# phazei/ComfyUI-HunyuanVideo-Foley

Measured on AMD Instinct MI355X. Metric: audio-sec/sec (5s clip, 50-step Euler, CFG 4.5), higher is better.
Workload: dtype bf16; 1 GPU; c2: T2A 5 s, 50 Euler steps, CFG 4.5, hunyuanvideo-foley-xxl, bs=1/GPU, bf16 GEMM operands / fp32 accumulate, weight storage none, DAC-VAE fp32 decode to 48 kHz, host-to-host (H2D noise + D2H waveform timed); clips_per_gpu=1, parallelism=dp1, hip_graph=True, progress_callback=False, collectives=0, bundle_bytes=10565004032, rccl_nranks=1

## Files before the change

comfyui-hunyuanvideo-foley_amd/csrc/common.h:

```cpp
#pragma once
#include <hip/hip_runtime.h>
#include <hip/hip_ext.h>
#include <stdint.h>

#include <atomic>

typedef __attribute__((ext_vector_type(16))) float f32x16;
typedef __attribute__((ext_vector_type(4))) float f32x4;
typedef __attribute__((ext_vector_type(8))) __bf16 bf16x8;
typedef __attribute__((ext_vector_type(4))) unsigned int u32x4;
typedef uint16_t bf16_t;
typedef _Float16 f16_t;
typedef __attribute__((ext_vector_type(8))) _Float16 f16x8;

enum { FOLEY_F32 = 0, FOLEY_BF16 = 1, FOLEY_I32 = 2, FOLEY_F8E4M3 = 3, FOLEY_F8E5M2 = 4, FOLEY_F16 = 5 };
__host__ __device__ constexpr bool foley_is_half(int dt) { return dt == FOLEY_BF16 || dt == FOLEY_F16; }

__device__ __forceinline__ float bf16_to_f32(bf16_t v) { return __uint_as_float(((uint32_t)v) << 16); }
__device__ __forceinline__ bf16_t f32_to_bf16(float f) {
  uint32_t u = __float_as_uint(f);
  if ((u & 0x7fffffffu) > 0x7f800000u) return (bf16_t)((u >> 16) | 0x40);
  u += 0x7fffu + ((u >> 16) & 1u);
  return (bf16_t)(u >> 16);
}
// ... 108 lines not shown
  float scale;
  int per;
  int dense_from;
  int dense_base;
};

__host__ __device__ __forceinline__ int rb_nearest_exact(int l, float scale, int Ls) {
  const int s = (int)floorf(((float)l + 0.5f) * scale);
  return s < Ls ? s : Ls - 1;
}

__device__ __forceinline__ const float* rb_row(const RowBcast& b, int r) {
  const float* p = b.p;
  if (b.step_ptr) p += (long)(*b.step_ptr) * b.step_stride;
  if (b.mode == 1) p += ((long)(r / b.rows_per_cfg) * b.L + (r % b.L)) * b.ld;
  else if (b.mode == 2) {
    const int s = rb_nearest_exact(r % b.L, b.scale, b.Ls), cfg = r / b.rows_per_cfg;
    const int idx = cfg < b.dense_from ? cfg * b.per + (s & (b.per - 1)) : b.dense_base + (cfg - b.dense_from) * b.Ls + s;
    p += (long)idx * b.ld;
  }
  return p;
}

struct FoleyProfHook {
  hipEvent_t e0, e1;
  const void* fn;
};
extern thread_local FoleyProfHook g_foley_prof;
#define FOLEY_LAUNCH(kernel, grid, block, lds, st, ...)                                                          \
  do {                                                                                                           \
    if (g_foley_prof.e0) {                                                                                       \
      hipExtLaunchKernelGGL(kernel, grid, block, lds, st, g_foley_prof.e0, g_foley_prof.e1, 0, __VA_ARGS__);     \
      g_foley_prof.e0 = nullptr;                                                                                 \
      g_foley_prof.fn = (const void*)(kernel);                                                                   \
    } else {                                                                                                     \
      hipLaunchKernelGGL(kernel, grid, block, lds, st, __VA_ARGS__);                                             \
    }                                                                                                            \
  } while (0)

#define FOLEY_CHECK_HIP(expr)                                         \
  do {                                                                \
    hipError_t _e = (expr);                                           \
    if (_e != hipSuccess) return foley_set_err(hipGetErrorString(_e), __FILE__, __LINE__); \
  } while (0)

int foley_set_err(const char* msg, const char* file, int line);
// ... 10 lines not shown
```

comfyui-hunyuanvideo-foley_amd/csrc/foley_rt.hip:

```cpp
#include "../../include/foley_hip.h"
#include "kernels.h"
#include "gemm_plan.h"

#include <algorithm>
#include <climits>
#include <cmath>
#include <cstdio>
#include <cstdlib>
#include <cstring>
#include <cxxabi.h>
#include <atomic>
#include <mutex>
#include <string>
#include <type_traits>
#include <unordered_map>
#include <vector>

thread_local FoleyProfHook g_foley_prof = {nullptr, nullptr};

static std::mutex g_setup_mutex;

static thread_local std::string g_err;
int foley_set_err(const char* msg, const char* file, int line) {
  const char* base = strrchr(file, '/');
// ... 1633 lines not shown
                     {Cout}, &an));
      GemmArgs g = gemm_plain(S_in, clips * Tout, down, X, Cout);
      g.lda = C; g.segV = Tout; g.segS = Tin; g.taps = 2 * s; g.tapC = C; g.dil = 1; g.tap0 = -pad; g.rstride = s;
      g.out1 = S_alt; g.alpha = (const float*)an; g.alphaC = Cout;
      TRY(launch_gemm(g, FOLEY_F32, EPI_DAC, 0, st));
      std::swap(S_in, S_alt);
    }
    Tin = Tout;
    C = Cout;
  }
  {
    Lin co, qc;
    TRY(get_lin(c, "enc.out", FOLEY_F32, L, 3 * C, true, &co));
    TRY(get_lin(c, "enc.qc", FOLEY_F32, 2 * L, L, true, &qc));
    TRY(launch_gemm(gemm_conv(S_in, clips * Tin, Tin, C, 3, 1, co, Z0, L), FOLEY_F32, EPI_STORE_F32, 0, st));
    TRY(launch_gemm(gemm_plain(Z0, clips * Tin, qc, Z1, 2 * L), FOLEY_F32, EPI_STORE_F32, 0, st));
    TRY(launch_rows_to_planes(Z1, clips, Tin, 2 * L, params, st));
  }
  HIPTRY(hipEventRecord(c->ev1, st));
  c->timed = true;
  return 0;
}

static RowBcast to_rb(const foley_rowbcast* r) {
  if (!r || !r->p) return rb_none();
  const int L = r->L > 0 ? r->L : 1, Ls = r->mode == 2 ? (r->Ls > 0 ? r->Ls : 1) : 0;
  const int per = (r->mode == 2 && r->period > 0 && !(r->period & (r->period - 1))) ? r->period : 0;
  RowBcast b{r->p, (long)r->ld, r->mode, r->rows_per_cfg > 0 ? r->rows_per_cfg : 1, L, nullptr, 0, Ls, Ls ? (float)Ls / (float)L : 0.f, per, 0, 0};
  if (per > 0) {
    b.dense_from = r->periodic_cfgs > 0 ? r->periodic_cfgs : INT_MAX;
    b.dense_base = r->periodic_cfgs > 0 ? r->periodic_cfgs * per : 0;
  }
  return b;
}

static int gemm_args_of(const foley_gemm_desc* d, GemmArgs& g) {
  if (!d) return FAIL(FOLEY_ERR_INVALID, "null descriptor");
  g = GemmArgs{};
  g.A = d->A; g.W = d->W; g.bias = d->bias; g.M = d->M; g.N = d->N; g.K = d->K; g.lda = d->lda;
  g.segV = d->segV; g.segS = d->segS; g.taps = d->taps; g.tapC = d->tapC; g.dil = d->dil; g.tap0 = d->tap0;
  g.out0 = d->out0; g.out1 = d->out1; g.osegV = d->osegV; g.out_seg = d->out_seg; g.out_row = d->out_row;
  g.out_shift = d->out_shift; g.out_check = d->out_check; g.rb = to_rb(&d->rb); g.res = d->res;
  g.alpha = d->alpha; g.alphaC = d->alphaC > 0 ? d->alphaC : 1;
  g.ksplit = d->ksplit;
  g.rstride = d->rstride;
  g.ldw = d->ldw;
  g.wfmt = d->wfmt;
  g.gelu_erf = d->gelu_erf;
  if (d->partials) {
    if (d->partial_slabs < 1) return FAIL(FOLEY_ERR_INVALID, "partials need partial_slabs >= 1");
    g.partials = d->partials; g.partial_stride = (long)d->M * d->N; g.partial_cap = d->partial_slabs;
    g.partial_half = d->partial_dtype != 0;
    if (d->partial_dtype != 0 && d->partial_dtype != d->dtype) return FAIL(FOLEY_ERR_INVALID, "partial_dtype must be 0 (fp32) or the operand dtype");
  }
  if (g.segV < 1 || g.segS < 1 || g.osegV < 1 || g.taps < 1) return FAIL(FOLEY_ERR_INVALID, "bad GEMM descriptor");
  if (d->epilogue == EPI_QKV_SPLIT) {
// ... 248 lines not shown
extern "C" int foley_op_windows_stitch(const float* x, int clips, int n_win, int C, int L, int Ltot, const int32_t* starts,
                                       const float* weights, float* out, void* stream) {
  return launch_windows_stitch(x, clips, n_win, C, L, Ltot, starts, weights, out, (hipStream_t)stream);
}

extern "C" int foley_op_flow_mix(const float* noise, const float* x0, int x0_clips, int clips, int C, int L, float sigma,
                                 float* out, void* stream) {
  return launch_flow_mix(noise, x0, x0_clips, clips, C, L, sigma, out, (hipStream_t)stream);
}

extern "C" int foley_op_latent_rows(const float* x, int clips, int C, int L, int ncfg, void* out, int out_dtype,
                                    void* stream) {
  return launch_latent_rows(x, clips, C, L, ncfg, out, out_dtype, (hipStream_t)stream);
}

extern "C" int foley_op_dac_out(const float* s, const float* w, const float* bias, int B, int T, int C, float* out,
                                void* stream) {
  return launch_dac_out(s, w, bias, B, T, C, out, (hipStream_t)stream);
}

extern "C" int foley_op_rows_add_act(const float* a, const float* v, int R, int D, int act_silu, void* out, int out_dtype,
                                     void* stream) {
  if (!out || R < 1 || D < 1) return FAIL(FOLEY_ERR_INVALID, "rows_add_act: null output or empty problem");
  return launch_rows_add_act(a, v ? rb_vec(v, 0, nullptr) : rb_none(), R, D, act_silu ? 1 : 0, out, out_dtype, (hipStream_t)stream);
}

extern "C" int foley_op_add_periodic(const float* x, const float* pos, int R, int D, int period, void* out, int out_dtype,
                                     void* stream) {
  if (!x || !pos || !out || R < 1 || D < 1 || period < 1) return FAIL(FOLEY_ERR_INVALID, "add_periodic: null argument or empty problem");
  return launch_add_periodic(x, pos, R, D, period, out, out_dtype, (hipStream_t)stream);
}

extern "C" int foley_op_gather_rows(const float* src, const int32_t* idx, int n_idx, int groups, int src_rows, int D, float* out,
                                    void* stream) {
  if (!src || !idx || !out || n_idx < 1 || groups < 1 || src_rows < 1 || D < 1)
    return FAIL(FOLEY_ERR_INVALID, "gather_rows: null argument or empty problem");
  return launch_gather_rows(src, idx, n_idx, groups, src_rows, D, out, (hipStream_t)stream);
}

extern "C" int foley_op_cast(const void* src, int src_dtype, void* dst, int dst_dtype, long n, void* stream) {
  if (!src || !dst || n < 1) return FAIL(FOLEY_ERR_INVALID, "cast: null argument or empty problem");
  return launch_cast(src, src_dtype, dst, dst_dtype, n, (hipStream_t)stream);
}

extern "C" int foley_op_rows_periodic_check(const float* x, int groups, int rows, int period, int D, int32_t* flags, void* stream) {
  if (!x || !flags || groups < 1 || rows < 1 || period < 1 || D < 1)
    return FAIL(FOLEY_ERR_INVALID, "rows_periodic_check: null argument or empty problem");
// ... 41 lines not shown
```

comfyui-hunyuanvideo-foley_amd/csrc/rowops.hip:

```cpp
#include <type_traits>

#include "kernels.h"

namespace {

#define FOLEY_LAUNCH_CHECK()                                                             \
  do {                                                                                   \
    hipError_t _e = hipGetLastError();                                                   \
    if (_e != hipSuccess) return foley_set_err(hipGetErrorString(_e), __FILE__, __LINE__); \
  } while (0)

template <typename OutT> struct Pack4;
template <> struct Pack4<float> {
  static __device__ __forceinline__ void store(float* p, const f32x4 v) { *(f32x4*)p = v; }
};
template <> struct Pack4<bf16_t> {
  static __device__ __forceinline__ void store(bf16_t* p, const f32x4 v) {
    uint2 w;
    w.x = pack_bf16x2(v[0], v[1]);
    w.y = pack_bf16x2(v[2], v[3]);
    *(uint2*)p = w;
  }
};

template <> struct Pack4<f16_t> {
  static __device__ __forceinline__ void store(f16_t* p, const f32x4 v) {
    uint2 w;
    w.x = pack_f16x2(v[0], v[1]);
    w.y = pack_f16x2(v[2], v[3]);
    *(uint2*)p = w;
  }
};

template <typename ST> __device__ __forceinline__ f32x4 slab_load4(const void* base, long elem) {
  if constexpr (sizeof(ST) == 4) {
    return *(const f32x4*)((const float*)base + elem);
  } else {
    const uint2 w = *(const uint2*)((const ST*)base + elem);
    const ST* h = (const ST*)&w;
    f32x4 v = {Cvt<ST>::from(h[0]), Cvt<ST>::from(h[1]), Cvt<ST>::from(h[2]), Cvt<ST>::from(h[3])};
    return v;
  }
}

struct LnPair {
  LnArgs a[2];
  int blocks0;
  long long* dbg;
};
static long long* g_ln_dbg = nullptr;
extern "C" void foley_debug_ln_timeline(void* p) { g_ln_dbg = (long long*)p; }

template <typename OutT, int MAXV, bool PEND, bool SLAB16 = false>
__global__ __launch_bounds__(128) void ln_mod_kernel(const LnPair pr, int D, float eps) {
  using ST = typename std::conditional<SLAB16, OutT, float>::type;
  const int sel = (int)blockIdx.x >= pr.blocks0 ? 1 : 0;
  const LnArgs& A = pr.a[sel];
  float* __restrict__ x = A.x;
  const int M = A.M;
  const RowBcast& shift = A.shift;
  const RowBcast& scale = A.scale;
  OutT* __restrict__ out = (OutT*)A.out;
  const int row = ((int)blockIdx.x - (sel ? pr.blocks0 : 0)) * 2 + (threadIdx.x >> 6);
  const int lane = threadIdx.x & 63;
  if (row >= M) return;
  const int nv = D >> 2;
  f32x4* xr = (f32x4*)(x + (long)row * D);
  const f32x4* sh = shift.p ? (const f32x4*)rb_row(shift, row) : nullptr;
  const f32x4* sc = scale.p ? (const f32x4*)rb_row(scale, row) : nullptr;
  const f32x4 z4 = {0.f, 0.f, 0.f, 0.f};
  f32x4 v[MAXV], hv[MAXV], cv[MAXV];
#pragma unroll
  for (int i = 0; i < MAXV; ++i) {
    const int c = min(lane + i * 64, nv - 1);
    v[i] = xr[c];
    hv[i] = sh ? sh[c] : z4;
    cv[i] = sc ? sc[c] : z4;
// ... 47 lines not shown
#pragma unroll
      for (int u = 0; u < 4; ++u) {
        const float d = v[i][u] - mean;
        q += d * d;
      }
    }
  const float rstd = 1.0f / sqrtf(wave_sum(q) / (float)D + eps);
  OutT* orow = out + (long)row * D;
#pragma unroll
  for (int i = 0; i < MAXV; ++i) {
    const int c = lane + i * 64;
    if (c < nv) {
      f32x4 y;
#pragma unroll
      for (int u = 0; u < 4; ++u) y[u] = (v[i][u] - mean) * rstd * (1.0f + cv[i][u]) + hv[i][u];
      Pack4<OutT>::store(orow + c * 4, y);
    }
  }
}

#ifndef FOLEY_LN_RPB
#define FOLEY_LN_RPB 1
#endif
template <typename OutT, int MAXV, bool PEND, int WPR, int SEL, bool SLAB16>
__device__ __forceinline__ void ln_mod_wide_body(const LnPair& pr, int D, float eps) {
  using ST = typename std::conditional<SLAB16, OutT, float>::type;
  constexpr int RPB = FOLEY_LN_RPB;
  __shared__ float red[RPB][2][WPR];
  constexpr int sel = SEL;
  const LnArgs& A = pr.a[SEL];
  const int M = A.M;
  const int wave = threadIdx.x >> 6, lane = threadIdx.x & 63;
  const int rb = wave / WPR, part = wave % WPR;
  const int row_u = ((int)blockIdx.x - (sel ? pr.blocks0 : 0)) * RPB + rb;
  const bool live = row_u < M;
  const int row = live ? row_u : M - 1;
  const int c0 = part * (MAXV * 64) + lane;
  const bool stamp = pr.dbg && threadIdx.x == 0;
  if (stamp) pr.dbg[(long)blockIdx.x * 4 + 0] = wall_clock64();
  f32x4* xr = (f32x4*)(A.x + (long)row * D);
  const f32x4* sh = A.shift.p ? (const f32x4*)rb_row(A.shift, row) : nullptr;
  const f32x4* sc = A.scale.p ? (const f32x4*)rb_row(A.scale, row) : nullptr;
  const f32x4 z4 = {0.f, 0.f, 0.f, 0.f};
  f32x4 v[MAXV], hv[MAXV], cv[MAXV];
#pragma unroll
  for (int i = 0; i < MAXV; ++i) {
    const int c = c0 + i * 64;
    v[i] = xr[c];
    hv[i] = sh ? sh[c] : z4;
    cv[i] = sc ? sc[c] : z4;
  }
  if (PEND && A.pend.partials) {
    constexpr int SB = 6;
    const LnPending& P = A.pend;
    const f32x4* gp = (const f32x4*)rb_row(P.gate, row);
    const f32x4* bp = (const f32x4*)P.bias;
    f32x4 acc[MAXV], gt[MAXV];
#pragma unroll
    for (int i = 0; i < MAXV; ++i) {
      const int c = c0 + i * 64;
      gt[i] = gp[c];
      acc[i] = bp ? bp[c] : z4;
// ... 3 lines not shown
#pragma unroll
      for (int u = 0; u < SB; ++u) {
        const int s = min(s0 + u, P.k - 1);
        const long pe = s * P.stride + (long)row * D;
#pragma unroll
        for (int i = 0; i < MAXV; ++i) t[u][i] = slab_load4<ST>(P.partials, pe + 4L * (c0 + i * 64));
      }
#pragma unroll
      for (int u = 0; u < SB; ++u) {
        const float w = (s0 + u < P.k) ? 1.0f : 0.0f;
#pragma unroll
        for (int i = 0; i < MAXV; ++i)
#pragma unroll
          for (int e = 0; e < 4; ++e) acc[i][e] += w * t[u][i][e];
      }
    }
#pragma unroll
    for (int i = 0; i < MAXV; ++i) {
#pragma unroll
      for (int e = 0; e < 4; ++e) v[i][e] += gt[i][e] * acc[i][e];
      if (live) xr[c0 + i * 64] = v[i];
    }
  }
  if (pr.dbg) {
    asm volatile("s_waitcnt vmcnt(0)" ::: "memory");
    if (stamp) pr.dbg[(long)blockIdx.x * 4 + 1] = wall_clock64();
  }
  float s = 0.f;
#pragma unroll
  for (int i = 0; i < MAXV; ++i) s += (v[i][0] + v[i][1]) + (v[i][2] + v[i][3]);
  s = wave_sum(s);
  const float nw = (float)(MAXV * 4 * 64);
  const float mean_w = s / nw;
  float q = 0.f;
#pragma unroll
  for (int i = 0; i < MAXV; ++i)
#pragma unroll
    for (int u = 0; u < 4; ++u) {
      const float d = v[i][u] - mean_w;
      q += d * d;
    }
  q = wave_sum(q);
  if (lane == 0) {
    red[rb][0][part] = s;
    red[rb][1][part] = q;
  }
  __syncthreads();
  float tot = 0.f;
#pragma unroll
  for (int w = 0; w < WPR; ++w) tot += red[rb][0][w];
  const float mean = tot / (float)D;
  float qt = 0.f;
#pragma unroll
  for (int w = 0; w < WPR; ++w) {
    const float dm = red[rb][0][w] / nw - mean;
    qt += red[rb][1][w] + nw * dm * dm;
  }
  const float rstd = 1.0f / sqrtf(qt / (float)D + eps);
  if (stamp) pr.dbg[(long)blockIdx.x * 4 + 2] = wall_clock64();
  if (!live) return;
  OutT* orow = (OutT*)A.out + (long)row * D;
#pragma unroll
  for (int i = 0; i < MAXV; ++i) {
    f32x4 y;
#pragma unroll
    for (int u = 0; u < 4; ++u) y[u] = (v[i][u] - mean) * rstd * (1.0f + cv[i][u]) + hv[i][u];
    Pack4<OutT>::store(orow + (c0 + i * 64) * 4, y);
  }
  if (stamp) pr.dbg[(long)blockIdx.x * 4 + 3] = wall_clock64();
}

template <typename OutT, int MAXV, bool PEND, int WPR, bool SLAB16 = false>
__global__ __launch_bounds__(64 * FOLEY_LN_RPB * WPR) void ln_mod_wide_kernel(const LnPair pr, int D, float eps) {
  if ((int)blockIdx.x >= pr.blocks0) ln_mod_wide_body<OutT, MAXV, PEND, WPR, 1, SLAB16>(pr, D, eps);
  else ln_mod_wide_body<OutT, MAXV, PEND, WPR, 0, SLAB16>(pr, D, eps);
}

struct QkvPair {
  QkvSplitArgs a[2];
  int blocks0;
};

template <typename OutT>
__global__ __launch_bounds__(256) void qkv_split_kernel(const QkvPair pr) {
  __shared__ OutT vt[32][128 + 2];
  const int sel = (int)blockIdx.x >= pr.blocks0 ? 1 : 0;
  const QkvSplitArgs& a = pr.a[sel];
  int bid = (int)blockIdx.x - (sel ? pr.blocks0 : 0);
  const bool vtrans = a.vt_pitch > 0;
  const int nQ = a.nK - (vtrans ? 1 : 0);
  const int lane = threadIdx.x & 63;
  constexpr int IPW = 4;
  const long n_items = (long)a.M * a.H * nQ;
  const int bqk = (int)((n_items + 4 * IPW - 1) / (4 * IPW));
  if (bid < bqk) {
    const long it0 = ((long)bid * 4 + (threadIdx.x >> 6)) * IPW;
    if (it0 >= n_items) return;
    float x0[IPW], x1[IPW];
// ... 48 lines not shown
#pragma unroll
    for (int i = 0; i < 4; ++i) {
      const int lr = r0 + i * 8;
      const int l = l0 + min(lr, nrows - 1);
      const f32x4 v = *(const f32x4*)(a.qkv + ((long)b * a.L + l) * (a.nK * a.H * 128) + (long)w * a.H * 128 +
                                      h * 128 + c4 * 4);
      vt[lr][c4 * 4 + 0] = Cvt<OutT>::to(v[0]);
      vt[lr][c4 * 4 + 1] = Cvt<OutT>::to(v[1]);
      vt[lr][c4 * 4 + 2] = Cvt<OutT>::to(v[2]);
      vt[lr][c4 * 4 + 3] = Cvt<OutT>::to(v[3]);
    }
  }
  __syncthreads();
  const int d = threadIdx.x >> 1, half = threadIdx.x & 1;
  OutT* dst = (OutT*)a.dst[w] + (((long)b * a.H + h) * 128 + d) * a.vt_pitch + a.tok_off + l0 + half * 16;
#pragma unroll
  for (int t = 0; t < 16; ++t)
    if (half * 16 + t < nrows) dst[t] = vt[half * 16 + t][d];
}

template <typename OutT>
__global__ void rows_add_act_kernel(const float* __restrict__ a, RowBcast v, int R, int D, int act_silu,
                                    OutT* __restrict__ out) {
  const long n = (long)R * D;
  const float* vr = v.p ? rb_row(v, 0) : nullptr;
  for (long i = (long)blockIdx.x * blockDim.x + threadIdx.x; i < n; i += (long)gridDim.x * blockDim.x) {
    float y = a ? a[i] : 0.f;
    if (vr) y += vr[i % D];
    if (act_silu) y = silu_f(y);
    out[i] = Cvt<OutT>::to(y);
  }
}

template <typename OutT>
__global__ void add_periodic_kernel(const float* __restrict__ x, const float* __restrict__ pos, int R, int D,
                                    int period, OutT* __restrict__ out) {
  const long n = (long)R * D;
  for (long i = (long)blockIdx.x * blockDim.x + threadIdx.x; i < n; i += (long)gridDim.x * blockDim.x) {
    const int r = (int)(i / D), c = (int)(i - (long)r * D);
    out[i] = Cvt<OutT>::to(x[i] + pos[(long)(r % period) * D + c]);
  }
}

__global__ void gather_rows_kernel(const float* __restrict__ src, const int* __restrict__ idx, int n_idx,
                                   int groups, int src_rows, int D, float* __restrict__ out) {
  const long n = (long)groups * n_idx * D;
  for (long i = (long)blockIdx.x * blockDim.x + threadIdx.x; i < n; i += (long)gridDim.x * blockDim.x) {
    const long r = i / D;
// ... 519 lines not shown
    const long b = bc / C;
    out[i] = rows[(b * T + t) * C + c];
  }
}

inline int grid1d(long n, int block) {
  long g = (n + block - 1) / block;
  return (int)(g > 4096 ? 4096 : (g < 1 ? 1 : g));
}

}

int launch_ln_mod_pair(const LnArgs& a0, const LnArgs& a1, int D, float eps, int out_dtype, hipStream_t st) {
  if (D % 4 || D > 8 * 256) return foley_set_err("ln_mod: D must be a multiple of 4 and <= 2048", __FILE__, __LINE__);
  for (const LnArgs* a : {&a0, &a1})
    if (a->M > 0 && a->pend.partials &&
        (a->pend.k < 1 || a->pend.stride % 4 || ((uintptr_t)a->pend.partials & 15) || ((uintptr_t)a->pend.bias & 15) ||
         !a->pend.gate.p || ((uintptr_t)a->pend.gate.p & 15) || a->pend.gate.ld % 4 || a->pend.gate.step_stride % 4))
      return foley_set_err("ln_mod: bad pending split-K descriptor", __FILE__, __LINE__);
  LnPair pr;
  pr.a[0] = a0;
  pr.a[1] = a1;
  pr.blocks0 = (a0.M + 1) / 2;
  pr.dbg = g_ln_dbg;
  dim3 grid(pr.blocks0 + (a1.M + 1) / 2), block(128);
  const int need = (D / 4 + 63) / 64;
  if (out_dtype != FOLEY_F32 && !foley_is_half(out_dtype)) return foley_set_err("ln_mod: bad dtype", __FILE__, __LINE__);
  const bool f32o = out_dtype == FOLEY_F32, f16o = out_dtype == FOLEY_F16;
  const bool pend = (a0.M > 0 && a0.pend.partials) || (a1.M > 0 && a1.pend.partials);
  const int h0 = (a0.M > 0 && a0.pend.partials) ? a0.pend.half : -1, h1 = (a1.M > 0 && a1.pend.partials) ? a1.pend.half : -1;
  const int slab_dt = h0 >= 0 ? h0 : (h1 >= 0 ? h1 : 0);
  if ((h0 >= 0 && h1 >= 0 && h0 != h1) || (slab_dt != 0 && slab_dt != out_dtype))
    return foley_set_err("ln_mod: 16-bit pending slabs must have the output dtype (and agree between the two row sets)", __FILE__, __LINE__);
  const bool s16 = slab_dt != 0;
#define FOLEY_LN(V)                                                                                        \
  {                                                                                                        \
    if (pend) {                                                                                            \
      if (f32o) FOLEY_LAUNCH((ln_mod_kernel<float, V, true>), grid, block, 0, st, pr, D, eps);       \
      else if (f16o && s16) FOLEY_LAUNCH((ln_mod_kernel<f16_t, V, true, true>), grid, block, 0, st, pr, D, eps);  \
      else if (f16o) FOLEY_LAUNCH((ln_mod_kernel<f16_t, V, true>), grid, block, 0, st, pr, D, eps);  \
      else if (s16) FOLEY_LAUNCH((ln_mod_kernel<bf16_t, V, true, true>), grid, block, 0, st, pr, D, eps);  \
      else FOLEY_LAUNCH((ln_mod_kernel<bf16_t, V, true>), grid, block, 0, st, pr, D, eps);           \
    } else {                                                                                               \
      if (f32o) FOLEY_LAUNCH((ln_mod_kernel<float, V, false>), grid, block, 0, st, pr, D, eps);      \
      else if (f16o) FOLEY_LAUNCH((ln_mod_kernel<f16_t, V, false>), grid, block, 0, st, pr, D, eps); \
      else FOLEY_LAUNCH((ln_mod_kernel<bf16_t, V, false>), grid, block, 0, st, pr, D, eps);          \
    }                                                                                                      \
  }
  const int total_rows = a0.M + a1.M;
  if (total_rows <= 4096 && D % (4 * 64 * 2) == 0 && D / (4 * 64 * 2) <= 4) {
    LnPair prw = pr;
    prw.blocks0 = (a0.M + FOLEY_LN_RPB - 1) / FOLEY_LN_RPB;
    const dim3 gridw(prw.blocks0 + (a1.M + FOLEY_LN_RPB - 1) / FOLEY_LN_RPB), blk(64 * FOLEY_LN_RPB * 2);
#define FOLEY_LNW(V)                                                                                                  \
    {                                                                                                                  \
      if (pend) {                                                                                                      \
        if (f32o) FOLEY_LAUNCH((ln_mod_wide_kernel<float, V, true, 2>), gridw, blk, 0, st, prw, D, eps);                \
        else if (f16o && s16) FOLEY_LAUNCH((ln_mod_wide_kernel<f16_t, V, true, 2, true>), gridw, blk, 0, st, prw, D, eps);  \
        else if (f16o) FOLEY_LAUNCH((ln_mod_wide_kernel<f16_t, V, true, 2>), gridw, blk, 0, st, prw, D, eps);           \
        else if (s16) FOLEY_LAUNCH((ln_mod_wide_kernel<bf16_t, V, true, 2, true>), gridw, blk, 0, st, prw, D, eps);     \
        else FOLEY_LAUNCH((ln_mod_wide_kernel<bf16_t, V, true, 2>), gridw, blk, 0, st, prw, D, eps);                    \
      } else {                                                                                                         \
        if (f32o) FOLEY_LAUNCH((ln_mod_wide_kernel<float, V, false, 2>), gridw, blk, 0, st, prw, D, eps);               \
        else if (f16o) FOLEY_LAUNCH((ln_mod_wide_kernel<f16_t, V, false, 2>), gridw, blk, 0, st, prw, D, eps);          \
        else FOLEY_LAUNCH((ln_mod_wide_kernel<bf16_t, V, false, 2>), gridw, blk, 0, st, prw, D, eps);                   \
      }                                                                                                                \
    }
    const int v2 = D / (4 * 64 * 2);
    if (v2 == 1) FOLEY_LNW(1)
    else if (v2 == 2) FOLEY_LNW(2)
    else if (v2 == 3) FOLEY_LNW(3)
    else FOLEY_LNW(4)
    FOLEY_LAUNCH_CHECK();
    return 0;
  }
#undef FOLEY_LNW
  if (need <= 2) FOLEY_LN(2)
  else if (need <= 4) FOLEY_LN(4)
  else if (need <= 6) FOLEY_LN(6)
  else FOLEY_LN(8)
#undef FOLEY_LN
  FOLEY_LAUNCH_CHECK();
  return 0;
}

int launch_ln_mod(const float* x, int M, int D, float eps, const RowBcast& shift, const RowBcast& scale,
                  void* out, int out_dtype, hipStream_t st) {
  LnArgs a0{const_cast<float*>(x), M, shift, scale, out, LnPending{}};
  LnArgs a1 = a0;
  a1.M = 0;
  return launch_ln_mod_pair(a0, a1, D, eps, out_dtype, st);
}

int launch_ln_mod_pending(float* x, int M, int D, float eps, const RowBcast& shift, const RowBcast& scale,
                          void* out, int out_dtype, const LnPending& pend, hipStream_t st) {
  LnArgs a0{x, M, shift, scale, out, pend};
  LnArgs a1 = a0;
  a1.M = 0;
  return launch_ln_mod_pair(a0, a1, D, eps, out_dtype, st);
}

int launch_qkv_split_pair(const QkvSplitArgs& a0, const QkvSplitArgs& a1, hipStream_t st) {
  if (a0.out_dtype != a1.out_dtype) return foley_set_err("qkv_split pair: dtype mismatch", __FILE__, __LINE__);
  QkvPair pr;
// ... 372 lines not shown
```

Baseline: 13.88 audio-sec/sec.

## Resolve row-broadcast maps on host and overlap step-index scalar load in LN kernels

Adds a resolved LayerNorm-modulation path. When shift, scale and gate share one row mapping and step pointer, the host packs them into a flat LnRes with raw pointers and a single RowMap. The kernel then issues the step-index scalar load early through inline s_load asm and waits on it only after the x and partial-slab loads have started. It also batches the partial-slab loads six at a time to raise memory-level parallelism. The old per-operand rb_row kernels remain as a fallback, and a debug hook for the step pointer plus a timeline-probe variant are added. The trade-offs are more template instantiations and fragile inline asm whose correctness depends on register constraints.

```diff
diff --git a/comfyui-hunyuanvideo-foley_amd/csrc/common.h b/comfyui-hunyuanvideo-foley_amd/csrc/common.h
--- a/comfyui-hunyuanvideo-foley_amd/csrc/common.h
+++ b/comfyui-hunyuanvideo-foley_amd/csrc/common.h
@@ -154,6 +154,54 @@
   return p;
 }
 
+struct RowMap {
+  long ld, step_stride;
+  int mode, rows_per_cfg, L, Ls;
+  float scale;
+  int per, dense_from, dense_base;
+};
+inline RowMap rb_map_of(const RowBcast& b) { return RowMap{b.ld, b.step_ptr ? b.step_stride : 0, b.mode, b.rows_per_cfg, b.L, b.Ls, b.scale, b.per, b.dense_from, b.dense_base}; }
+inline bool rb_map_equal(const RowMap& a, const RowMap& b) {
+  return a.ld == b.ld && a.step_stride == b.step_stride && a.mode == b.mode && a.rows_per_cfg == b.rows_per_cfg && a.L == b.L && a.Ls == b.Ls &&
+         a.scale == b.scale && a.per == b.per && a.dense_from == b.dense_from && a.dense_base == b.dense_base;
+}
+inline bool rb_resolvable(const RowBcast* const* ops, int n, const int** step_ptr, RowMap* map) {
+  bool first = true;
+  *map = RowMap{0, 0, 0, 1, 1, 0, 0.f, 0, 0, 0};
+  for (int i = 0; i < n; ++i) {
+    const RowBcast& b = *ops[i];
+    if (!b.p) continue;
+    if (b.step_ptr) {
+      if (*step_ptr && *step_ptr != b.step_ptr) return false;
+      *step_ptr = b.step_ptr;
+    }
+    const RowMap m = rb_map_of(b);
+    if (first) *map = m;
+    else if (!rb_map_equal(*map, m)) return false;
+    first = false;
+  }
+  return true;
+}
+
+__device__ __forceinline__ int rb_step_load(const int* __restrict__ step_ptr) { return step_ptr ? *step_ptr : 0; }
+
+__device__ __forceinline__ const float* rb_row_at(const RowBcast& b, int step, int r) {
+  RowBcast c = b;
+  c.step_ptr = nullptr;
+  return rb_row(c, r) + (b.step_ptr ? (long)step * b.step_stride : 0L);
+}
+
+__device__ __forceinline__ long rb_map_off(const RowMap& m, int step, int r) {
+  long off = (long)step * m.step_stride;
+  if (m.mode == 1) off += ((long)(r / m.rows_per_cfg) * m.L + (r % m.L)) * m.ld;
+  else if (m.mode == 2) {
+    const int s = rb_nearest_exact(r % m.L, m.scale, m.Ls), cfg = r / m.rows_per_cfg;
+    const int idx = cfg < m.dense_from ? cfg * m.per + (s & (m.per - 1)) : m.dense_base + (cfg - m.dense_from) * m.Ls + s;
+    off += (long)idx * m.ld;
+  }
+  return off;
+}
+
 struct FoleyProfHook {
   hipEvent_t e0, e1;
   const void* fn;
diff --git a/comfyui-hunyuanvideo-foley_amd/csrc/foley_rt.hip b/comfyui-hunyuanvideo-foley_amd/csrc/foley_rt.hip
--- a/comfyui-hunyuanvideo-foley_amd/csrc/foley_rt.hip
+++ b/comfyui-hunyuanvideo-foley_amd/csrc/foley_rt.hip
@@ -1679,6 +1679,23 @@
   return 0;
 }
 
+static thread_local const int* g_rb_step_ptr[2] = {nullptr, nullptr};
+static thread_local long g_rb_step_stride = 0;
+static thread_local unsigned g_rb_step_n = 0;
+extern "C" void foley_debug_rowbcast_step(const int32_t* p0, const int32_t* p1, int64_t step_stride) {
+  g_rb_step_ptr[0] = p0;
+  g_rb_step_ptr[1] = p1 ? p1 : p0;
+  g_rb_step_stride = (long)step_stride;
+  g_rb_step_n = 0;
+}
+static RowBcast rb_debug_step(RowBcast b) {
+  if (b.p && g_rb_step_ptr[0]) {
+    b.step_ptr = g_rb_step_ptr[g_rb_step_n++ & 1];
+    b.step_stride = g_rb_step_stride;
+  }
+  return b;
+}
+
 static RowBcast to_rb(const foley_rowbcast* r) {
   if (!r || !r->p) return rb_none();
   const int L = r->L > 0 ? r->L : 1, Ls = r->mode == 2 ? (r->Ls > 0 ? r->Ls : 1) : 0;
@@ -1688,7 +1705,7 @@
     b.dense_from = r->periodic_cfgs > 0 ? r->periodic_cfgs : INT_MAX;
     b.dense_base = r->periodic_cfgs > 0 ? r->periodic_cfgs * per : 0;
   }
-  return b;
+  return rb_debug_step(b);
 }
 
 static int gemm_args_of(const foley_gemm_desc* d, GemmArgs& g) {
@@ -1983,7 +2000,7 @@
 extern "C" int foley_op_rows_add_act(const float* a, const float* v, int R, int D, int act_silu, void* out, int out_dtype,
                                      void* stream) {
   if (!out || R < 1 || D < 1) return FAIL(FOLEY_ERR_INVALID, "rows_add_act: null output or empty problem");
-  return launch_rows_add_act(a, v ? rb_vec(v, 0, nullptr) : rb_none(), R, D, act_silu ? 1 : 0, out, out_dtype, (hipStream_t)stream);
+  return launch_rows_add_act(a, v ? rb_debug_step(rb_vec(v, 0, nullptr)) : rb_none(), R, D, act_silu ? 1 : 0, out, out_dtype, (hipStream_t)stream);
 }
 
 extern "C" int foley_op_add_periodic(const float* x, const float* pos, int R, int D, int period, void* out, int out_dtype,
diff --git a/comfyui-hunyuanvideo-foley_amd/csrc/rowops.hip b/comfyui-hunyuanvideo-foley_amd/csrc/rowops.hip
--- a/comfyui-hunyuanvideo-foley_amd/csrc/rowops.hip
+++ b/comfyui-hunyuanvideo-foley_amd/csrc/rowops.hip
@@ -46,13 +46,161 @@
 struct LnPair {
   LnArgs a[2];
   int blocks0;
-  long long* dbg;
 };
 static long long* g_ln_dbg = nullptr;
 extern "C" void foley_debug_ln_timeline(void* p) { g_ln_dbg = (long long*)p; }
 
+struct LnRes {
+  float* x;
+  void* out;
+  const float *shift, *scale, *gate;
+  const float *partials, *bias;
+  long pstride;
+  int M, k;
+  RowMap map;
+};
+struct LnResPair {
+  const int* step_ptr;
+  int blocks0;
+  LnRes a[2];
+  long long* dbg;
+};
+
+template <typename ST> struct SlabRaw { using type = f32x4; };
+template <> struct SlabRaw<bf16_t> { using type = uint2; };
+template <> struct SlabRaw<f16_t> { using type = uint2; };
+template <typename ST> __device__ __forceinline__ f32x4 slab_cvt4(const typename SlabRaw<ST>::type& w) {
+  if constexpr (sizeof(ST) == 4) {
+    return w;
+  } else {
+    const ST* h = (const ST*)&w;
+    f32x4 v = {Cvt<ST>::from(h[0]), Cvt<ST>::from(h[1]), Cvt<ST>::from(h[2]), Cvt<ST>::from(h[3])};
+    return v;
+  }
+}
+template <typename ST, int MAXV, int SB, typename ColFn>
+__device__ __forceinline__ void slab_batch_load(typename SlabRaw<ST>::type (&t)[SB][MAXV], const void* partials, long pstride, int k, int s0, long row_elem,
+                                                ColFn col) {
+#pragma unroll
+  for (int u = 0; u < SB; ++u) {
+    const int s = min(s0 + u, k - 1);
+    const long pe = s * pstride + row_elem;
+#pragma unroll
+    for (int i = 0; i < MAXV; ++i) t[u][i] = *(const typename SlabRaw<ST>::type*)((const ST*)partials + pe + 4L * col(i));
+  }
+}
+template <typename ST, int MAXV, int SB>
+__device__ __forceinline__ void slab_batch_add(f32x4 (&acc)[MAXV], const typename SlabRaw<ST>::type (&t)[SB][MAXV], int k, int s0) {
+#pragma unroll
+  for (int u = 0; u < SB; ++u) {
+    const float w = (s0 + u < k) ? 1.0f : 0.0f;
+#pragma unroll
+    for (int i = 0; i < MAXV; ++i) {
+      const f32x4 tv = slab_cvt4<ST>(t[u][i]);
+#pragma unroll
+      for (int e = 0; e < 4; ++e) acc[i][e] += w * tv[e];
+    }
+  }
+}
+
+__device__ __forceinline__ int ln_step_issue(const LnRes& A, const int* step_ptr) {
+  int v;
+  asm volatile("s_load_dword %0, %1, 0x0"
+               : "=&s"(v)
+               : "s"(step_ptr), "s"(A.x), "s"(A.out), "s"(A.shift), "s"(A.scale), "s"(A.gate), "s"(A.partials), "s"(A.bias), "s"(A.pstride), "s"(A.M), "s"(A.k),
+                 "s"(A.map.ld), "s"(A.map.step_stride), "s"(A.map.mode), "s"(A.map.rows_per_cfg), "s"(A.map.L), "s"(A.map.Ls), "s"(A.map.scale),
+                 "s"(A.map.per), "s"(A.map.dense_from), "s"(A.map.dense_base));
+  return v;
+}
+__device__ __forceinline__ int ln_step_wait(int v) {
+  asm volatile("s_waitcnt lgkmcnt(0)" : "+s"(v));
+  return v;
+}
+
 template <typename OutT, int MAXV, bool PEND, bool SLAB16 = false>
-__global__ __launch_bounds__(128) void ln_mod_kernel(const LnPair pr, int D, float eps) {
+__global__ __launch_bounds__(128) void ln_mod_kernel(const LnResPair pr, int D, float eps) {
+  using ST = typename std::conditional<SLAB16, OutT, float>::type;
+  constexpr int SB = 6;
+  const int sel = (int)blockIdx.x >= pr.blocks0 ? 1 : 0;
+  const LnRes& A = pr.a[sel];
+  const int step_sent = ln_step_issue(A, pr.step_ptr);
+  const int M = A.M;
+  OutT* __restrict__ out = (OutT*)A.out;
+  const int row = ((int)blockIdx.x - (sel ? pr.blocks0 : 0)) * 2 + (threadIdx.x >> 6);
+  const int lane = threadIdx.x & 63;
+  if (row >= M) return;
+  const int nv = D >> 2;
+  f32x4* xr = (f32x4*)(A.x + (long)row * D);
+  const f32x4 z4 = {0.f, 0.f, 0.f, 0.f};
+  const bool pend = PEND && A.partials;
+  const auto col = [&](int i) { return min(lane + i * 64, nv - 1); };
+  f32x4 v[MAXV], hv[MAXV], cv[MAXV], acc[MAXV], gt[MAXV];
+  typename SlabRaw<ST>::type t[PEND ? SB : 1][MAXV];
+#pragma unroll
+  for (int i = 0; i < MAXV; ++i) v[i] = xr[col(i)];
+  if (pend) {
+    const f32x4* bp = (const f32x4*)A.bias;
+#pragma unroll
+    for (int i = 0; i < MAXV; ++i) acc[i] = bp ? bp[col(i)] : z4;
+    if constexpr (PEND) slab_batch_load<ST, MAXV, SB>(t, A.partials, A.pstride, A.k, 0, (long)row * D, col);
+  }
+  const long row_off = rb_map_off(A.map, 0, row);
+  const long off = row_off + (long)ln_step_wait(step_sent) * A.map.step_stride;
+  const f32x4* sh = A.shift ? (const f32x4*)(A.shift + off) : nullptr;
+  const f32x4* sc = A.scale ? (const f32x4*)(A.scale + off) : nullptr;
+#pragma unroll
+  for (int i = 0; i < MAXV; ++i) {
+    hv[i] = sh ? sh[col(i)] : z4;
+    cv[i] = sc ? sc[col(i)] : z4;
+  }
+  if constexpr (PEND) {
+    if (pend) {
+      const f32x4* gp = (const f32x4*)(A.gate + off);
+#pragma unroll
+      for (int i = 0; i < MAXV; ++i) gt[i] = gp[col(i)];
+      for (int s0 = 0; s0 < A.k; s0 += SB) {
+        if (s0 > 0) slab_batch_load<ST, MAXV, SB>(t, A.partials, A.pstride, A.k, s0, (long)row * D, col);
+        slab_batch_add<ST, MAXV, SB>(acc, t, A.k, s0);
+      }
+#pragma unroll
+      for (int i = 0; i < MAXV; ++i) {
+#pragma unroll
+        for (int e = 0; e < 4; ++e) v[i][e] += gt[i][e] * acc[i][e];
+        if (lane + i * 64 < nv) xr[lane + i * 64] = v[i];
+      }
+    }
+  }
+  float s = 0.f;
+#pragma unroll
+  for (int i = 0; i < MAXV; ++i)
+    if (lane + i * 64 < nv) s += (v[i][0] + v[i][1]) + (v[i][2] + v[i][3]);
+  const float mean = wave_sum(s) / (float)D;
+  float q = 0.f;
+#pragma unroll
+  for (int i = 0; i < MAXV; ++i)
+    if (lane + i * 64 < nv) {
+#pragma unroll
+      for (int u = 0; u < 4; ++u) {
+        const float d = v[i][u] - mean;
+        q += d * d;
+      }
+    }
+  const float rstd = 1.0f / sqrtf(wave_sum(q) / (float)D + eps);
+  OutT* orow = out + (long)row * D;
+#pragma unroll
+  for (int i = 0; i < MAXV; ++i) {
+    const int c = lane + i * 64;
+    if (c < nv) {
+      f32x4 y;
+#pragma unroll
+      for (int u = 0; u < 4; ++u) y[u] = (v[i][u] - mean) * rstd * (1.0f + cv[i][u]) + hv[i][u];
+      Pack4<OutT>::store(orow + c * 4, y);
+    }
+  }
+}
+
+template <typename OutT, int MAXV, bool PEND, bool SLAB16 = false>
+__global__ __launch_bounds__(128) void ln_mod_each_kernel(const LnPair pr, int D, float eps) {
   using ST = typename std::conditional<SLAB16, OutT, float>::type;
   const int sel = (int)blockIdx.x >= pr.blocks0 ? 1 : 0;
   const LnArgs& A = pr.a[sel];
@@ -146,11 +294,127 @@
 #ifndef FOLEY_LN_RPB
 #define FOLEY_LN_RPB 1
 #endif
+template <typename OutT, int MAXV, int WPR, bool STAMP>
+__device__ __forceinline__ void ln_wide_finish(const f32x4 (&v)[MAXV], const f32x4 (&hv)[MAXV], const f32x4 (&cv)[MAXV], OutT* orow, int c0, int rb,
+                                               int part, int lane, bool live, int D, float eps, long long* stamps) {
+  __shared__ float red[FOLEY_LN_RPB][2][WPR];
+  float s = 0.f;
+#pragma unroll
+  for (int i = 0; i < MAXV; ++i) s += (v[i][0] + v[i][1]) + (v[i][2] + v[i][3]);
+  s = wave_sum(s);
+  const float nw = (float)(MAXV * 4 * 64);
+  const float mean_w = s / nw;
+  float q = 0.f;
+#pragma unroll
+  for (int i = 0; i < MAXV; ++i)
+#pragma unroll
+    for (int u = 0; u < 4; ++u) {
+      const float d = v[i][u] - mean_w;
+      q += d * d;
+    }
+  q = wave_sum(q);
+  if (lane == 0) {
+    red[rb][0][part] = s;
+    red[rb][1][part] = q;
+  }
+  __syncthreads();
+  float tot = 0.f;
+#pragma unroll
+  for (int w = 0; w < WPR; ++w) tot += red[rb][0][w];
+  const float mean = tot / (float)D;
+  float qt = 0.f;
+#pragma unroll
+  for (int w = 0; w < WPR; ++w) {
+    const float dm = red[rb][0][w] / nw - mean;
+    qt += red[rb][1][w] + nw * dm * dm;
+  }
+  const float rstd = 1.0f / sqrtf(qt / (float)D + eps);
+  if (STAMP && stamps) stamps[2] = wall_clock64();
+  if (!live) return;
+#pragma unroll
+  for (int i = 0; i < MAXV; ++i) {
+    f32x4 y;
+#pragma unroll
+    for (int u = 0; u < 4; ++u) y[u] = (v[i][u] - mean) * rstd * (1.0f + cv[i][u]) + hv[i][u];
+    Pack4<OutT>::store(orow + (c0 + i * 64) * 4, y);
+  }
+  if (STAMP && stamps) stamps[3] = wall_clock64();
+}
+
+template <typename OutT, int MAXV, bool PEND, int WPR, int SEL, bool SLAB16, bool DBG>
+__device__ __forceinline__ void ln_mod_wide_body(const LnResPair& pr, int D, float eps) {
+  using ST = typename std::conditional<SLAB16, OutT, float>::type;
+  constexpr int RPB = FOLEY_LN_RPB, SB = 6;
+  const LnRes& A = pr.a[SEL];
+  const int M = A.M;
+  const int wave = threadIdx.x >> 6, lane = threadIdx.x & 63;
+  const int rb = wave / WPR, part = wave % WPR;
+  const int row_u = ((int)blockIdx.x - (SEL ? pr.blocks0 : 0)) * RPB + rb;
+  const bool live = row_u < M;
+  const int row = live ? row_u : M - 1;
+  const int c0 = part * (MAXV * 64) + lane;
+  long long* const stamps = (DBG && threadIdx.x == 0) ? pr.dbg + (long)blockIdx.x * 4 : nullptr;
+  if (DBG && stamps) stamps[0] = wall_clock64();
+  f32x4* xr = (f32x4*)(A.x + (long)row * D);
+  const f32x4 z4 = {0.f, 0.f, 0.f, 0.f};
+  const bool pend = PEND && A.partials;
+  const auto col = [&](int i) { return c0 + i * 64; };
+  f32x4 v[MAXV], hv[MAXV], cv[MAXV], acc[MAXV], gt[MAXV];
+  typename SlabRaw<ST>::type t[PEND ? SB : 1][MAXV];
+  const int step_sent = ln_step_issue(A, pr.step_ptr);
+#pragma unroll
+  for (int i = 0; i < MAXV; ++i) v[i] = xr[col(i)];
+  if constexpr (PEND) {
+    if (pend) {
+      const f32x4* bp = (const f32x4*)A.bias;
+#pragma unroll
+      for (int i = 0; i < MAXV; ++i) acc[i] = bp ? bp[col(i)] : z4;
+      slab_batch_load<ST, MAXV, SB>(t, A.partials, A.pstride, A.k, 0, (long)row * D, col);
+    }
+  }
+  const long row_off = rb_map_off(A.map, 0, row);
+  const long off = row_off + (long)ln_step_wait(step_sent) * A.map.step_stride;
+  const f32x4* sh = A.shift ? (const f32x4*)(A.shift + off) : nullptr;
+  const f32x4* sc = A.scale ? (const f32x4*)(A.scale + off) : nullptr;
+#pragma unroll
+  for (int i = 0; i < MAXV; ++i) {
+    hv[i] = sh ? sh[col(i)] : z4;
+    cv[i] = sc ? sc[col(i)] : z4;
+  }
+  if constexpr (PEND) {
+    if (pend) {
+      const f32x4* gp = (const f32x4*)(A.gate + off);
+#pragma unroll
+      for (int i = 0; i < MAXV; ++i) gt[i] = gp[col(i)];
+      for (int s0 = 0; s0 < A.k; s0 += SB) {
+        if (s0 > 0) slab_batch_load<ST, MAXV, SB>(t, A.partials, A.pstride, A.k, s0, (long)row * D, col);
+        slab_batch_add<ST, MAXV, SB>(acc, t, A.k, s0);
+      }
+#pragma unroll
+      for (int i = 0; i < MAXV; ++i) {
+#pragma unroll
+        for (int e = 0; e < 4; ++e) v[i][e] += gt[i][e] * acc[i][e];
+        if (live) xr[col(i)] = v[i];
+      }
+    }
+  }
+  if (DBG) {
+    asm volatile("s_waitcnt vmcnt(0)" ::: "memory");
+    if (stamps) stamps[1] = wall_clock64();
+  }
+  ln_wide_finish<OutT, MAXV, WPR, DBG>(v, hv, cv, (OutT*)A.out + (long)row * D, c0, rb, part, lane, live, D, eps, stamps);
+}
+
+template <typename OutT, int MAXV, bool PEND, int WPR, bool SLAB16 = false, bool DBG = false>
+__global__ __launch_bounds__(64 * FOLEY_LN_RPB * WPR) void ln_mod_wide_kernel(const LnResPair pr, int D, float eps) {
+  if ((int)blockIdx.x >= pr.blocks0) ln_mod_wide_body<OutT, MAXV, PEND, WPR, 1, SLAB16, DBG>(pr, D, eps);
+  else ln_mod_wide_body<OutT, MAXV, PEND, WPR, 0, SLAB16, DBG>(pr, D, eps);
+}
+
 template <typename OutT, int MAXV, bool PEND, int WPR, int SEL, bool SLAB16>
-__device__ __forceinline__ void ln_mod_wide_body(const LnPair& pr, int D, float eps) {
+__device__ __forceinline__ void ln_mod_wide_each_body(const LnPair& pr, int D, float eps) {
   using ST = typename std::conditional<SLAB16, OutT, float>::type;
   constexpr int RPB = FOLEY_LN_RPB;
-  __shared__ float red[RPB][2][WPR];
   constexpr int sel = SEL;
   const LnArgs& A = pr.a[SEL];
   const int M = A.M;
@@ -160,8 +424,6 @@
   const bool live = row_u < M;
   const int row = live ? row_u : M - 1;
   const int c0 = part * (MAXV * 64) + lane;
-  const bool stamp = pr.dbg && threadIdx.x == 0;
-  if (stamp) pr.dbg[(long)blockIdx.x * 4 + 0] = wall_clock64();
   f32x4* xr = (f32x4*)(A.x + (long)row * D);
   const f32x4* sh = A.shift.p ? (const f32x4*)rb_row(A.shift, row) : nullptr;
   const f32x4* sc = A.scale.p ? (const f32x4*)rb_row(A.scale, row) : nullptr;
@@ -211,58 +473,13 @@
       if (live) xr[c0 + i * 64] = v[i];
     }
   }
-  if (pr.dbg) {
-    asm volatile("s_waitcnt vmcnt(0)" ::: "memory");
-    if (stamp) pr.dbg[(long)blockIdx.x * 4 + 1] = wall_clock64();
-  }
-  float s = 0.f;
-#pragma unroll
-  for (int i = 0; i < MAXV; ++i) s += (v[i][0] + v[i][1]) + (v[i][2] + v[i][3]);
-  s = wave_sum(s);
-  const float nw = (float)(MAXV * 4 * 64);
-  const float mean_w = s / nw;
-  float q = 0.f;
-#pragma unroll
-  for (int i = 0; i < MAXV; ++i)
-#pragma unroll
-    for (int u = 0; u < 4; ++u) {
-      const float d = v[i][u] - mean_w;
-      q += d * d;
-    }
-  q = wave_sum(q);
-  if (lane == 0) {
-    red[rb][0][part] = s;
-    red[rb][1][part] = q;
-  }
-  __syncthreads();
-  float tot = 0.f;
-#pragma unroll
-  for (int w = 0; w < WPR; ++w) tot += red[rb][0][w];
-  const float mean = tot / (float)D;
-  float qt = 0.f;
-#pragma unroll
-  for (int w = 0; w < WPR; ++w) {
-    const float dm = red[rb][0][w] / nw - mean;
-    qt += red[rb][1][w] + nw * dm * dm;
-  }
-  const float rstd = 1.0f / sqrtf(qt / (float)D + eps);
-  if (stamp) pr.dbg[(long)blockIdx.x * 4 + 2] = wall_clock64();
-  if (!live) return;
-  OutT* orow = (OutT*)A.out + (long)row * D;
-#pragma unroll
-  for (int i = 0; i < MAXV; ++i) {
-    f32x4 y;
-#pragma unroll
-    for (int u = 0; u < 4; ++u) y[u] = (v[i][u] - mean) * rstd * (1.0f + cv[i][u]) + hv[i][u];
-    Pack4<OutT>::store(orow + (c0 + i * 64) * 4, y);
-  }
-  if (stamp) pr.dbg[(long)blockIdx.x * 4 + 3] = wall_clock64();
+  ln_wide_finish<OutT, MAXV, WPR, false>(v, hv, cv, (OutT*)A.out + (long)row * D, c0, rb, part, lane, live, D, eps, nullptr);
 }
 
 template <typename OutT, int MAXV, bool PEND, int WPR, bool SLAB16 = false>
-__global__ __launch_bounds__(64 * FOLEY_LN_RPB * WPR) void ln_mod_wide_kernel(const LnPair pr, int D, float eps) {
-  if ((int)blockIdx.x >= pr.blocks0) ln_mod_wide_body<OutT, MAXV, PEND, WPR, 1, SLAB16>(pr, D, eps);
-  else ln_mod_wide_body<OutT, MAXV, PEND, WPR, 0, SLAB16>(pr, D, eps);
+__global__ __launch_bounds__(64 * FOLEY_LN_RPB * WPR) void ln_mod_wide_each_kernel(const LnPair pr, int D, float eps) {
+  if ((int)blockIdx.x >= pr.blocks0) ln_mod_wide_each_body<OutT, MAXV, PEND, WPR, 1, SLAB16>(pr, D, eps);
+  else ln_mod_wide_each_body<OutT, MAXV, PEND, WPR, 0, SLAB16>(pr, D, eps);
 }
 
 struct QkvPair {
@@ -357,8 +574,9 @@
 template <typename OutT>
 __global__ void rows_add_act_kernel(const float* __restrict__ a, RowBcast v, int R, int D, int act_silu,
                                     OutT* __restrict__ out) {
+  const int step = rb_step_load(v.p ? v.step_ptr : nullptr);
   const long n = (long)R * D;
-  const float* vr = v.p ? rb_row(v, 0) : nullptr;
+  const float* vr = v.p ? rb_row_at(v, step, 0) : nullptr;
   for (long i = (long)blockIdx.x * blockDim.x + threadIdx.x; i < n; i += (long)gridDim.x * blockDim.x) {
     float y = a ? a[i] : 0.f;
     if (vr) y += vr[i % D];
@@ -924,7 +1142,21 @@
   pr.a[0] = a0;
   pr.a[1] = a1;
   pr.blocks0 = (a0.M + 1) / 2;
-  pr.dbg = g_ln_dbg;
+  LnResPair rp{};
+  bool resolved = true;
+  for (int i = 0; i < 2; ++i) {
+    const LnArgs& a = pr.a[i];
+    const bool pd = a.M > 0 && a.pend.partials;
+    LnRes& r = rp.a[i];
+    r = LnRes{a.x, a.out, a.shift.p, a.scale.p, pd ? a.pend.gate.p : nullptr, pd ? a.pend.partials : nullptr, pd ? a.pend.bias : nullptr,
+              pd ? a.pend.stride : 0, a.M, pd ? a.pend.k : 0, RowMap{}};
+    const RowBcast none{};
+    const RowBcast* ops[3] = {&a.shift, &a.scale, pd ? &a.pend.gate : &none};
+    if (a.M > 0 && !rb_resolvable(ops, 3, &rp.step_ptr, &r.map)) resolved = false;
+  }
+  if (!rp.step_ptr) rp.step_ptr = (const int*)(a0.M > 0 ? a0.x : a1.x);
+  rp.blocks0 = pr.blocks0;
+  rp.dbg = g_ln_dbg;
   dim3 grid(pr.blocks0 + (a1.M + 1) / 2), block(128);
   const int need = (D / 4 + 63) / 64;
   if (out_dtype != FOLEY_F32 && !foley_is_half(out_dtype)) return foley_set_err("ln_mod: bad dtype", __FILE__, __LINE__);
@@ -935,53 +1167,69 @@
   if ((h0 >= 0 && h1 >= 0 && h0 != h1) || (slab_dt != 0 && slab_dt != out_dtype))
     return foley_set_err("ln_mod: 16-bit pending slabs must have the output dtype (and agree between the two row sets)", __FILE__, __LINE__);
   const bool s16 = slab_dt != 0;
-#define FOLEY_LN(V)                                                                                        \
-  {                                                                                                        \
-    if (pend) {                                                                                            \
-      if (f32o) FOLEY_LAUNCH((ln_mod_kernel<float, V, true>), grid, block, 0, st, pr, D, eps);       \
-      else if (f16o && s16) FOLEY_LAUNCH((ln_mod_kernel<f16_t, V, true, true>), grid, block, 0, st, pr, D, eps);  \
-      else if (f16o) FOLEY_LAUNCH((ln_mod_kernel<f16_t, V, true>), grid, block, 0, st, pr, D, eps);  \
-      else if (s16) FOLEY_LAUNCH((ln_mod_kernel<bf16_t, V, true, true>), grid, block, 0, st, pr, D, eps);  \
-      else FOLEY_LAUNCH((ln_mod_kernel<bf16_t, V, true>), grid, block, 0, st, pr, D, eps);           \
-    } else {                                                                                               \
-      if (f32o) FOLEY_LAUNCH((ln_mod_kernel<float, V, false>), grid, block, 0, st, pr, D, eps);      \
-      else if (f16o) FOLEY_LAUNCH((ln_mod_kernel<f16_t, V, false>), grid, block, 0, st, pr, D, eps); \
-      else FOLEY_LAUNCH((ln_mod_kernel<bf16_t, V, false>), grid, block, 0, st, pr, D, eps);          \
-    }                                                                                                      \
+#define FOLEY_LN_PEND(K, P, G, B, ...)                                                         \
+  {                                                                                            \
+    if (f32o) FOLEY_LAUNCH((K<float, __VA_ARGS__>), G, B, 0, st, P, D, eps);                   \
+    else if (f16o && s16) FOLEY_LAUNCH((K<f16_t, __VA_ARGS__, true>), G, B, 0, st, P, D, eps); \
+    else if (f16o) FOLEY_LAUNCH((K<f16_t, __VA_ARGS__>), G, B, 0, st, P, D, eps);              \
+    else if (s16) FOLEY_LAUNCH((K<bf16_t, __VA_ARGS__, true>), G, B, 0, st, P, D, eps);        \
+    else FOLEY_LAUNCH((K<bf16_t, __VA_ARGS__>), G, B, 0, st, P, D, eps);                       \
+  }
+#define FOLEY_LN_PLAIN(K, P, G, B, ...)                                                          \
+  {                                                                                              \
+    if (f32o) FOLEY_LAUNCH((K<float, __VA_ARGS__>), G, B, 0, st, P, D, eps);                     \
+    else if (f16o) FOLEY_LAUNCH((K<f16_t, __VA_ARGS__>), G, B, 0, st, P, D, eps);                \
+    else FOLEY_LAUNCH((K<bf16_t, __VA_ARGS__>), G, B, 0, st, P, D, eps);                         \
+  }
+#define FOLEY_LN_ANY(K, P, G, B, V, ...)                           \
+  {                                                                \
+    if (pend) FOLEY_LN_PEND(K, P, G, B, V, true, ##__VA_ARGS__)    \
+    else FOLEY_LN_PLAIN(K, P, G, B, V, false, ##__VA_ARGS__)       \
   }
   const int total_rows = a0.M + a1.M;
-  if (total_rows <= 4096 && D % (4 * 64 * 2) == 0 && D / (4 * 64 * 2) <= 4) {
+  const bool wide = total_rows <= 4096 && D % (4 * 64 * 2) == 0 && D / (4 * 64 * 2) <= 4;
+  if (rp.dbg) {
+    if (!(resolved && wide && out_dtype == FOLEY_BF16 && D == 1536))
+      return foley_set_err("ln_mod: the timeline probe is built for the resolved two-wave kernel, bf16 output, D = 1536", __FILE__, __LINE__);
+    rp.blocks0 = (a0.M + FOLEY_LN_RPB - 1) / FOLEY_LN_RPB;
+    const dim3 gridw(rp.blocks0 + (a1.M + FOLEY_LN_RPB - 1) / FOLEY_LN_RPB), blk(64 * FOLEY_LN_RPB * 2);
+    if (pend && s16) FOLEY_LAUNCH((ln_mod_wide_kernel<bf16_t, 3, true, 2, true, true>), gridw, blk, 0, st, rp, D, eps);
+    else if (pend) FOLEY_LAUNCH((ln_mod_wide_kernel<bf16_t, 3, true, 2, false, true>), gridw, blk, 0, st, rp, D, eps);
+    else FOLEY_LAUNCH((ln_mod_wide_kernel<bf16_t, 3, false, 2, false, true>), gridw, blk, 0, st, rp, D, eps);
+    FOLEY_LAUNCH_CHECK();
+    return 0;
+  }
+  if (wide) {
     LnPair prw = pr;
-    prw.blocks0 = (a0.M + FOLEY_LN_RPB - 1) / FOLEY_LN_RPB;
+    prw.blocks0 = rp.blocks0 = (a0.M + FOLEY_LN_RPB - 1) / FOLEY_LN_RPB;
     const dim3 gridw(prw.blocks0 + (a1.M + FOLEY_LN_RPB - 1) / FOLEY_LN_RPB), blk(64 * FOLEY_LN_RPB * 2);
-#define FOLEY_LNW(V)                                                                                                  \
-    {                                                                                                                  \
-      if (pend) {                                                                                                      \
-        if (f32o) FOLEY_LAUNCH((ln_mod_wide_kernel<float, V, true, 2>), gridw, blk, 0, st, prw, D, eps);                \
-        else if (f16o && s16) FOLEY_LAUNCH((ln_mod_wide_kernel<f16_t, V, true, 2, true>), gridw, blk, 0, st, prw, D, eps);  \
-        else if (f16o) FOLEY_LAUNCH((ln_mod_wide_kernel<f16_t, V, true, 2>), gridw, blk, 0, st, prw, D, eps);           \
-        else if (s16) FOLEY_LAUNCH((ln_mod_wide_kernel<bf16_t, V, true, 2, true>), gridw, blk, 0, st, prw, D, eps);     \
-        else FOLEY_LAUNCH((ln_mod_wide_kernel<bf16_t, V, true, 2>), gridw, blk, 0, st, prw, D, eps);                    \
-      } else {                                                                                                         \
-        if (f32o) FOLEY_LAUNCH((ln_mod_wide_kernel<float, V, false, 2>), gridw, blk, 0, st, prw, D, eps);               \
-        else if (f16o) FOLEY_LAUNCH((ln_mod_wide_kernel<f16_t, V, false, 2>), gridw, blk, 0, st, prw, D, eps);          \
-        else FOLEY_LAUNCH((ln_mod_wide_kernel<bf16_t, V, false, 2>), gridw, blk, 0, st, prw, D, eps);                   \
-      }                                                                                                                \
+#define FOLEY_LNW(V)                                                             \
+    {                                                                            \
+      if (resolved) FOLEY_LN_ANY(ln_mod_wide_kernel, rp, gridw, blk, V, 2)       \
+      else FOLEY_LN_ANY(ln_mod_wide_each_kernel, prw, gridw, blk, V, 2)          \
     }
     const int v2 = D / (4 * 64 * 2);
     if (v2 == 1) FOLEY_LNW(1)
     else if (v2 == 2) FOLEY_LNW(2)
     else if (v2 == 3) FOLEY_LNW(3)
     else FOLEY_LNW(4)
+#undef FOLEY_LNW
     FOLEY_LAUNCH_CHECK();
     return 0;
   }
-#undef FOLEY_LNW
-  if (need <= 2) FOLEY_LN(2)
-  else if (need <= 4) FOLEY_LN(4)
-  else if (need <= 6) FOLEY_LN(6)
-  else FOLEY_LN(8)
-#undef FOLEY_LN
+#define FOLEY_LNN(V)                                                             \
+  {                                                                              \
+    if (resolved) FOLEY_LN_ANY(ln_mod_kernel, rp, grid, block, V)                \
+    else FOLEY_LN_ANY(ln_mod_each_kernel, pr, grid, block, V)                    \
+  }
+  if (need <= 2) FOLEY_LNN(2)
+  else if (need <= 4) FOLEY_LNN(4)
+  else if (need <= 6) FOLEY_LNN(6)
+  else FOLEY_LNN(8)
+#undef FOLEY_LNN
+#undef FOLEY_LN_ANY
+#undef FOLEY_LN_PLAIN
+#undef FOLEY_LN_PEND
   FOLEY_LAUNCH_CHECK();
   return 0;
 }
```

Measured after the change: 14.13 audio-sec/sec, median of 6. 1.02x the previous value.
